# Yotsuei/ClearConverse

Measured on AMD Instinct MI355X. Metric: xRT (audio-sec/wall-sec) end-to-end, 30 s 16 kHz clips, higher is better.
Workload: dtype bf16

## Files before the change

clearconverse_amd/_lib.py:

```python
from __future__ import annotations

import ctypes as C
import os
from pathlib import Path
from typing import Optional

_PKG = Path(__file__).resolve().parent
LIB_PATH = _PKG / "libccx.so"


class CcxError(RuntimeError):
    pass


class WhisperDims(C.Structure):
    _fields_ = [(n, C.c_int) for n in (
        "n_mels", "n_audio_ctx", "n_audio_state", "n_audio_head", "n_audio_layer",
        "n_vocab", "n_text_ctx", "n_text_state", "n_text_head", "n_text_layer")]


class SepformerDims(C.Structure):
    _fields_ = [(n, C.c_int) for n in (
        "n_filters", "kernel", "stride", "d_model", "n_head", "d_ffn", "n_layers", "n_blocks", "segment", "n_spk")]

# ... 31 lines not shown
        ("rows", C.c_int), ("n_seq", C.c_int), ("H", C.c_int), ("kv_T", C.c_int), ("T", C.c_int),
        ("pos", C.POINTER(C.c_int)), ("row_seq", C.POINTER(C.c_int)), ("rows_per_seq", C.c_int),
        ("nsplit", C.c_int), ("combine", C.c_int), ("lds_pad", C.c_int),
        ("x", C.c_void_p), ("pend", C.c_void_p), ("pend_n", C.c_int), ("pend_stride", C.c_int64),
        ("ln_g", C.c_void_p), ("ln_b", C.c_void_p), ("eps", C.c_float),
        ("wq_host", C.c_void_p), ("bq", C.c_void_p),
        ("out", C.c_void_p), ("part_o", C.c_void_p), ("part_ml", C.c_void_p), ("q_x_out", C.c_void_p),
        ("q_elems", C.c_int64), ("kv_elems", C.c_int64), ("out_elems", C.c_int64), ("part_o_elems", C.c_int64),
        ("part_ml_elems", C.c_int64), ("x_elems", C.c_int64), ("pend_elems", C.c_int64), ("q_x_out_elems", C.c_int64),
        ("ind", C.POINTER(C.c_uint16)), ("ind_ld", C.c_int)]


DEC_ATTN_SELF, DEC_ATTN_SPLIT, DEC_ATTN_STREAM, DEC_ATTN_PREFILL, DEC_ATTN_FUSED_Q, DEC_ATTN_TWO_LAUNCH_Q = range(6)
DEC_ATTN_STREAM_MAPPED = 7
DEC_ATTN_SELF_IND = 8


class DecodeSamplingOptions(C.Structure):
    _fields_ = [("top_k", C.c_int), ("top_p", C.c_float), ("min_p", C.c_float)]


class DecSeqState(C.Structure):
    _fields_ = [(n, C.c_int) for n in ("pos", "prompt_len", "n_gen", "done", "last_tok", "pen_tok", "last_ts_tok", "n_tokens")] + [
        ("sum_logprob", C.c_float), ("no_speech_prob", C.c_float)]


class DecSelectDesc(C.Structure):
    _fields_ = [
        ("logits", C.c_void_p), ("ld", C.c_int64), ("n_vocab", C.c_int), ("B", C.c_int),
        ("rules", C.POINTER(DecodeRules)), ("state", C.POINTER(DecSeqState)),
# ... 208 lines not shown
    "ccx_whisper_set_history_options": (_i, [_vp, C.POINTER(DecodeHistoryOptions)]),
    "ccx_whisper_history_graph_count": (_i, [_vp]),
    "ccx_dec_history_step": (_i, [_vp, C.POINTER(DecHistoryDesc), _vp]),
    "ccx_decode_bias_options_default": (None, [C.POINTER(DecodeBiasOptions)]),
    "ccx_whisper_set_bias_options": (_i, [_vp, C.POINTER(DecodeBiasOptions)]),
    "ccx_whisper_bias_graph_count": (_i, [_vp]),
    "ccx_dec_bias_step": (_i, [_vp, C.POINTER(DecBiasDesc), _vp]),
    "ccx_decode_sampling_options_default": (None, [C.POINTER(DecodeSamplingOptions)]),
    "ccx_whisper_set_sampling_options": (_i, [_vp, C.POINTER(DecodeSamplingOptions)]),
    "ccx_whisper_sampling_graph_count": (_i, [_vp]),
    "ccx_whisper_set_mel": (_i, [_vp, _vp, _i, _vp]),
    "ccx_whisper_encode": (_i, [_vp, _i, _vp, _vp]),
    "ccx_whisper_decoder_logits": (_i, [_vp, _i32p, _i, _i, _vp, _vp]),
    "ccx_whisper_decode_greedy": (_i, [_vp, _i32p, _i32p, _i, _i, _i, _i32p, _i32p, _fp, _fp, _vp]),
    "ccx_dec_attention_desc": (_i, [_vp, _i, C.POINTER(DecAttnDesc), _vp]),
    "ccx_dec_select_step": (_i, [_vp, C.POINTER(DecSelectDesc), _vp]),
    "ccx_dec_beam_step": (_i, [_vp, C.POINTER(DecBeamDesc), _vp]),
    "ccx_whisper_decode_beam": (_i, [_vp, _i32p, _i32p, _i, _i, _i32p, _i, _i, _i, _i, _i32p, _i32p, _fp, _i32p, _fp,
                                     C.POINTER(BeamTrace), _vp]),
    "ccx_dec_token_probs": (_i, [_vp, C.POINTER(DecTokenProbsDesc), _vp]),
    "ccx_dec_pick_probs": (_i, [_vp, C.POINTER(DecPickProbsDesc), _vp]),
    "ccx_align_op": (_i, [_vp, _i, C.POINTER(AlignDesc), _vp]),
    "ccx_whisper_align": (_i, [_vp, _i32p, _i32p, _i, _i, _i32p, _i32p, _i, _i, _vp, _vp, _i32p, _vp]),
    "ccx_whisper_align_probs": (_i, [_vp, _i32p, _i32p, _i, _i, _i32p, _i32p, _i, _i, _vp, _vp, _i32p, _i, _fp, _vp]),
    "ccx_whisper_last_cross_path": (_i, [_vp]),
    "ccx_whisper_set_sot_tail": (_i, [_vp, _i]),
    "ccx_whisper_set_prefix_len": (_i, [_vp, _i]),
    "ccx_whisper_detect_language": (_i, [_vp, _i, _i, _i, _i32p, _fp, _vp]),
    "ccx_whisper_prepare_lanes": (_i, [_vp, _vp]),
    "ccx_whisper_trace_lanes": (_i, [_vp, C.c_char_p, _i]),
# ... 118 lines not shown
```

clearconverse_amd/csrc/dec_ops.hip:

```cpp
#include "../../include/ccx.h"
#include "ccx_common.h"
#include "decoder.h"
#include "op_scratch.h"

static_assert(sizeof(ccx_dec_seq_state) == sizeof(DecSeqState), "ccx_dec_seq_state mirrors DecSeqState field for field");

namespace {

__global__ void dec_ops_bf16_to_f32_kernel(const bf16_t* __restrict__ in, float* __restrict__ out, long n) {
  const long i = (long)blockIdx.x * 256 + threadIdx.x;
  if (i < n) out[i] = bf16_to_f32(in[i]);
}

}

extern "C" int ccx_dec_attention_desc(ccx_ctx* ctx, int form, const ccx_dec_attn_desc* d, void* stream_) {
  if (!ctx) return CCX_ERR_ARG;
  hipStream_t stream = (hipStream_t)stream_;
  CCX_REQUIRE(ctx, d != nullptr, "ccx_dec_attention_desc: desc is NULL");
  CCX_REQUIRE(ctx, (form >= CCX_DEC_ATTN_SELF && form <= CCX_DEC_ATTN_TWO_LAUNCH_Q) || form == CCX_DEC_ATTN_STREAM_MAPPED || form == CCX_DEC_ATTN_SELF_IND,
              "ccx_dec_attention_desc: unknown form %d", form);
  const bool is_ind = form == CCX_DEC_ATTN_SELF_IND;
  const bool is_self = form == CCX_DEC_ATTN_SELF || is_ind, is_split = form == CCX_DEC_ATTN_SPLIT, is_mapped = form == CCX_DEC_ATTN_STREAM_MAPPED,
             is_stream = form == CCX_DEC_ATTN_STREAM || is_mapped;
// ... 120 lines not shown
    rc = ccx_launch_dec_cross_fused_q(ctx, ap, rows, nsplit, stream);
  } else {
    DO_HIP(sc.alloc(&d_q, (size_t)rows * 768));
    DecLinearParams lp;
    memset(&lp, 0, sizeof(lp));
    lp.M = rows; lp.N = 768; lp.K = 768; lp.W = d_wq; lp.ldw = 768; lp.bias = (const float*)d->bq; lp.out = d_q; lp.ldo = 768;
    lp.x = (const float*)d->x; lp.pend = (const float*)d->pend; lp.pend_n = d->pend_n; lp.pend_stride = (long)d->pend_stride;
    lp.x_out = (float*)d->q_x_out; lp.ln_g = (const float*)d->ln_g; lp.ln_b = (const float*)d->ln_b; lp.eps = d->eps;
    rc = ccx_launch_dec_linear(ctx, ACT_LN, DEPI_F32, lp, stream);
    ap.q = d_q;
    if (rc == CCX_OK) rc = ccx_launch_dec_attention(ctx, ap, rows, nsplit, false, stream);
  }
  if (rc == CCX_OK && final_out) {
    hipLaunchKernelGGL(dec_ops_bf16_to_f32_kernel, dim3((unsigned)((n_out + 255) / 256)), dim3(256), 0, stream, d_out16, (float*)d->out, n_out);
    DO_HIP(hipGetLastError());
  }
  DO_HIP(hipStreamSynchronize(stream));
  return rc;
}

extern "C" int ccx_dec_select_step(ccx_ctx* ctx, const ccx_dec_select_desc* d, void* stream_) {
  if (!ctx) return CCX_ERR_ARG;
  hipStream_t stream = (hipStream_t)stream_;
  CCX_REQUIRE(ctx, d != nullptr, "ccx_dec_select_step: desc is NULL");
  const int V = d->n_vocab, B = d->B, D = d->D;
  CCX_REQUIRE(ctx, B >= 1 && B <= 65536, "ccx_dec_select_step: B = %d out of range", B);
  CCX_REQUIRE(ctx, V >= 4 && V % 4 == 0 && V <= 13 * 4096, "ccx_dec_select_step: n_vocab = %d must be a multiple of 4 and <= 53248", V);
  CCX_REQUIRE(ctx, d->ld >= V && d->ld % 4 == 0, "ccx_dec_select_step: ld = %ld must be >= n_vocab and a multiple of 4", (long)d->ld);
  CCX_REQUIRE(ctx, d->logits && ccx_aligned16(d->logits), "ccx_dec_select_step: logits null or not 16-byte aligned");
  CCX_REQUIRE(ctx, (int64_t)(B - 1) * d->ld + V <= d->logits_elems, "ccx_dec_select_step: logits are read up to element %ld, logits_elems=%ld",
// ... 226 lines not shown
```

clearconverse_amd/csrc/decoder.h:

```cpp
#pragma once
#include <cstring>
#include <vector>
#include "../../include/ccx.h"
#include "ccx_common.h"

enum { ACT_LN = 0, ACT_BF16 = 1, ACT_COMBINE = 2 };
enum { DEPI_BF16_GELU = 1, DEPI_PARTIAL = 2, DEPI_F32 = 3, DEPI_SELF_QKV = 4, DEPI_RESOLVE = 5 };

struct DecLinearParams {
  int M, N, K;
  const bf16_t* W; long ldw;
  const float* bias;
  const float* x;
  const float* pend; int pend_n; long pend_stride;
  float* x_out;
  const float* ln_g; const float* ln_b; float eps;
  float* ln_mean_out;
  const bf16_t* act; long lda;
  const float* part_o; const float* part_ml; int nsplit;
  float* xres; bf16_t* xb; float2* st_out; const float* shift; float shift_c;
  void* out; long ldo;
  bf16_t* cache_k; bf16_t* cache_v; int cache_T; const int* pos; const int* row_seq;
};
int ccx_launch_dec_linear(ccx_ctx* ctx, int act, int epi, const DecLinearParams& p, hipStream_t stream);
int ccx_dec_linear_ksplit(int K, int epi);
int ccx_launch_dec_resolve_ln(ccx_ctx* ctx, const float* x, const float* pend, int pend_n, long pend_stride, const float* g,
                              const float* b, bf16_t* out, float* x_out, int M, int K, float eps, hipStream_t stream,
                              float* mean_out = nullptr);

struct DecAttnParams {
  const float* q;
  const bf16_t* k;
  const bf16_t* v;
  int H, kv_T;
  const int* pos;
  int T;
  float scale_log2e;
  bf16_t* out_bf16;
  float* part_o;
  float* part_ml;
  int lds_pad;
  int stream_mode;
  const int* row_seq; int rows_per_seq;
// ... 172 lines not shown
```

clearconverse_amd/csrc/decoder.hip:

```cpp
#include <string>
#include "decoder.h"

__global__ void dec_embed_kernel(const float* __restrict__ tok_emb, const float* __restrict__ pos_emb,
                                 const int* __restrict__ cur_tok, const int* __restrict__ pos, float* __restrict__ x,
                                 int D) {
  const int b = blockIdx.x;
  const float4* te = (const float4*)(tok_emb + (long)cur_tok[b] * D);
  const float4* pe = (const float4*)(pos_emb + (long)pos[b] * D);
  float4* xo = (float4*)(x + (long)b * D);
  for (int i = threadIdx.x; i < D / 4; i += blockDim.x) {
    const float4 a = te[i], c = pe[i];
    xo[i] = make_float4(a.x + c.x, a.y + c.y, a.z + c.z, a.w + c.w);
  }
}

#include "dec_ln.h"

__device__ __forceinline__ float centre_shift(float mean, float rstd) { return fabsf(mean) * rstd > 1.f ? mean : 0.f; }

__device__ __forceinline__ uint4 combine_partials(const float* part_o, const float* part_ml, int nsplit, int mh, int c) {
  const float2* ml = (const float2*)(part_ml + ((long)mh * nsplit) * 2);
  const float* ob = part_o + ((long)mh * nsplit) * 64 + 8 * c;
  float2 mlv[8];
  float4 oa[8], oc[8];
// ... 89 lines not shown
  }

  bf16x8 wf[NT][KMAX];
#pragma unroll
  for (int i = 0; i < NT; i++) {
    const long tile = (long)(blockIdx.x * NT + i) * ksteps + ks0;
    const bf16_t* wr = p.W + (tile * 64 + lane) * 8;
#pragma unroll
    for (int k = 0; k < KMAX; k++) {
      const int kk = k < nks ? k : 0;
      wf[i][k] = __builtin_nontemporal_load((const bf16x8*)(wr + 512 * kk));
    }
  }
  bf16x8 af[MT][KMAX];
  if (BF16IN) {
#pragma unroll
    for (int j = 0; j < MT; j++) {
      int m = m0 + 16 * j + l15;
      m = m < p.M ? m : p.M - 1;
      const bf16_t* ar = p.act + (long)m * p.lda + 8 * h4 + 32 * ks0;
#pragma unroll
      for (int k = 0; k < KMAX; k++) {
        const int kk = k < nks ? k : 0;
        af[j][k] = *(const bf16x8*)(ar + 32 * kk);
      }
    }
  }

  if (ACT == ACT_LN) {
    const int nv = K >> 2;
    int live = p.M - m0;
    live = live > MROWS ? MROWS : live;
    const bool writer = (blockIdx.x == 0 && blockIdx.z == 0 && p.x_out != nullptr);
    float4 g[LNS], bb[LNS];
#pragma unroll
    for (int i = 0; i < LNS; i++) {
      const int idx = lane + 64 * i;
      const int ic = idx < nv ? idx : 0;
      g[i] = ((const float4*)p.ln_g)[ic];
// ... 119 lines not shown
        *(float4*)(p.xres + (long)m * p.N + n) = make_float4(v[0], v[1], v[2], v[3]);
        uint2 pk;
        pk.x = pack_bf16x2(c0, c1); pk.y = pack_bf16x2(c2, c3);
        *(uint2*)(p.xb + (long)m * p.N + n) = pk;
        if ((ln >> 4) == 0) p.st_out[(long)m * (p.N >> 4) + (n >> 4)] = make_float2(s1, s2);
      }
      continue;
    }
    if (n >= p.N || m >= p.M) continue;
    f32x4 v = *(const f32x4*)(red + (((0 * NT + i) * MT + j) * 64 + ln) * 4);
#pragma unroll
    for (int w = 1; w < NW; w++) v += *(const f32x4*)(red + (((w * NT + i) * MT + j) * 64 + ln) * 4);
    v[0] += bias_v[it].x; v[1] += bias_v[it].y; v[2] += bias_v[it].z; v[3] += bias_v[it].w;
    const bool full = n + 3 < p.N;
    if (EPI == DEPI_BF16_GELU) {
      bf16_t* o = (bf16_t*)p.out + (long)m * p.ldo + n;
      if (full) {
        uint2 pk;
        pk.x = pack_bf16x2(gelu_erf(v[0]), gelu_erf(v[1]));
        pk.y = pack_bf16x2(gelu_erf(v[2]), gelu_erf(v[3]));
        *(uint2*)o = pk;
      } else {
        for (int c = 0; c < 4 && n + c < p.N; c++) o[c] = f32_to_bf16(gelu_erf(v[c]));
      }
    } else if (EPI == DEPI_PARTIAL || EPI == DEPI_F32) {
      float* o = (float*)p.out + (EPI == DEPI_PARTIAL ? (long)blockIdx.z * p.pend_stride : 0L) + (long)m * p.ldo + n;
      if (full) *(float4*)o = make_float4(v[0], v[1], v[2], v[3]);
      else
        for (int c = 0; c < 4 && n + c < p.N; c++) o[c] = v[c];
    } else if (EPI == DEPI_SELF_QKV) {
      const int D = p.K;
// ... 8 lines not shown
        const int sq = p.row_seq ? p.row_seq[m] : m;
        uint2 pk;
        pk.x = pack_bf16x2(v[0], v[1]);
        pk.y = pack_bf16x2(v[2], v[3]);
        *(uint2*)(cache + (((long)sq * H + hh) * p.cache_T + pos_v[it]) * 64 + d) = pk;
      }
    }
  }
}

template <int NS>
__global__ __launch_bounds__(256) void dec_resolve_ln_kernel(const float* __restrict__ x, const float* __restrict__ pend,
                                                             int pend_n, long pend_stride, const float* __restrict__ g,
                                                             const float* __restrict__ b, bf16_t* __restrict__ out,
                                                             float* __restrict__ x_out, int M, int K, float eps,
                                                             float* __restrict__ mean_out) {
  const int lane = threadIdx.x & 63;
  const int m = blockIdx.x * 4 + (threadIdx.x >> 6);
  if (m >= M) return;
  const int nv = K >> 2;
  float4 v[NS], gg[NS], bb[NS];
#pragma unroll
  for (int i = 0; i < NS; i++) {
    const int idx = lane + 64 * i;
    const int ic = idx < nv ? idx : 0;
    gg[i] = ((const float4*)g)[ic];
    bb[i] = ((const float4*)b)[ic];
  }
  float sm = 0.f;
#pragma unroll
  for (int i = 0; i < NS; i++) {
// ... 10 lines not shown
    if (x_out && idx < nv) ((float4*)(x_out + (long)m * K))[idx] = a;
    sm += ln_sum4(a);
  }
  const float mean = wave_reduce_sum(sm) / (float)K;
  float sq = 0.f;
#pragma unroll
  for (int i = 0; i < NS; i++) {
    const float t = ln_sq4(v[i], mean);
    sq += (lane + 64 * i < nv) ? t : 0.f;
  }
  const float rstd = rsqrtf(wave_reduce_sum(sq) / (float)K + eps);
  if (mean_out && lane == 0) mean_out[m] = centre_shift(mean, rstd);
#pragma unroll
  for (int i = 0; i < NS; i++) {
    const int idx = lane + 64 * i;
    if (idx < nv) ((uint2*)(out + (long)m * K))[idx] = ln_pack4(v[i], mean, rstd, gg[i], bb[i]);
  }
}

__global__ __launch_bounds__(256) void dec_combine_kernel(const float* __restrict__ part_o, const float* __restrict__ part_ml,
                                                          int nsplit, bf16_t* __restrict__ out, int M, int H) {
  const int e = blockIdx.x * 256 + threadIdx.x;
  if (e >= M * H * 8) return;
  const int c = e & 7, h = (e >> 3) % H, m = e / (8 * H);
  *(uint4*)(out + ((long)m * H + h) * 64 + 8 * c) = combine_partials(part_o, part_ml, nsplit, m * H + h, c);
}

__global__ void dec_gather_rows_kernel(const bf16_t* __restrict__ src, const int* __restrict__ idx, bf16_t* __restrict__ dst, int D) {
  if (idx[blockIdx.x] < 0) return;
  const uint4* s4 = (const uint4*)(src + (long)idx[blockIdx.x] * D);
  uint4* d4 = (uint4*)(dst + (long)blockIdx.x * D);
// ... 6 lines not shown
  CCX_CHECK_LAUNCH(ctx);
  return CCX_OK;
}

int ccx_launch_dec_combine(ccx_ctx* ctx, const float* part_o, const float* part_ml, int nsplit, bf16_t* out, int M, int H,
                           hipStream_t stream) {
  CCX_REQUIRE(ctx, nsplit >= 1 && nsplit <= 8, "dec_combine: nsplit out of range");
  ccx_prof_scope ps(ctx, stream, "dec_combine_kernel", 0.0, (double)M * H * nsplit * 66.0 * 4 + (double)M * H * 64 * 2);
  hipLaunchKernelGGL(dec_combine_kernel, dim3(ccx_cdiv(M * H * 8, 256)), dim3(256), 0, stream, part_o, part_ml, nsplit, out, M, H);
  CCX_CHECK_LAUNCH(ctx);
  return CCX_OK;
}

int ccx_launch_dec_resolve_ln(ccx_ctx* ctx, const float* x, const float* pend, int pend_n, long pend_stride, const float* g,
                              const float* b, bf16_t* out, float* x_out, int M, int K, float eps, hipStream_t stream,
                              float* mean_out) {
  CCX_REQUIRE(ctx, K % 4 == 0 && K <= 1280, "dec_resolve_ln: K=%d unsupported (a multiple of 4, at most 1280)", K);
  CCX_REQUIRE(ctx, x_out != x, "dec_resolve_ln: x_out must not alias x");
  ccx_prof_scope ps(ctx, stream, "dec_resolve_ln_kernel", 0.0, (double)M * K * (4.0 * (1 + pend_n) + 2.0 + (x_out ? 4.0 : 0.0)));
  if (K <= 1024)
    hipLaunchKernelGGL(dec_resolve_ln_kernel<4>, dim3(ccx_cdiv(M, 4)), dim3(256), 0, stream, x, pend, pend_n, pend_stride, g, b,
                       out, x_out, M, K, eps, mean_out);
  else
    hipLaunchKernelGGL(dec_resolve_ln_kernel<5>, dim3(ccx_cdiv(M, 4)), dim3(256), 0, stream, x, pend, pend_n, pend_stride, g, b,
                       out, x_out, M, K, eps, mean_out);
  CCX_CHECK_LAUNCH(ctx);
  return CCX_OK;
}

template <int MT, int NT, int KMAX, int ACT, int EPI>
static int launch_dec_linear_inst(ccx_ctx* ctx, const DecLinearParams& p, int ksplit, hipStream_t stream) {
  const int MROWS = 16 * MT, BN = 16 * NT;
  size_t act_bytes = ACT == ACT_BF16 ? 0 : ccx_align((size_t)MROWS * (p.K + 8) * 2, 16);
  size_t red_bytes = (size_t)4 * NT * MT * 64 * 4 * 4;
  size_t lds = act_bytes + red_bytes;
  CCX_REQUIRE(ctx, lds <= 160 * 1024, "dec_linear: LDS %zu too large", lds);
  CCX_REQUIRE(ctx, ccx_cdiv(ccx_cdiv(p.K / 32, ksplit), 4) <= KMAX, "dec_linear: K=%d / split %d exceeds the prefetch depth %d", p.K, ksplit, KMAX);
  if (EPI == DEPI_RESOLVE) CCX_REQUIRE(ctx, p.xres && p.xb && p.st_out && ksplit == 1 && p.N % BN == 0, "dec_linear: bad resolve arguments (N=%d, %d columns per block)", p.N, BN);
  static ccx_lds_optin optin;
  if (lds > 64 * 1024) CCX_HIP(ctx, optin.ensure(ctx->device, (const void*)dec_linear_kernel<MT, NT, KMAX, ACT, EPI>));
// ... 16 lines not shown
  if (need <= 6) {
    if (M <= 16) return launch_dec_linear_inst<1, NT, 6, ACT, EPI>(ctx, p, ksplit, stream);
    if (M <= 32) return launch_dec_linear_inst<2, NT, 6, ACT, EPI>(ctx, p, ksplit, stream);
    return launch_dec_linear_inst<4, NT, 6, ACT, EPI>(ctx, p, ksplit, stream);
  }
  if (need <= 8) {
    if (M <= 16) return launch_dec_linear_inst<1, NT, 8, ACT, EPI>(ctx, p, ksplit, stream);
    if (M <= 32) return launch_dec_linear_inst<2, NT, 8, ACT, EPI>(ctx, p, ksplit, stream);
    return launch_dec_linear_inst<4, NT, 8, ACT, EPI>(ctx, p, ksplit, stream);
  }
  if (M <= 16) return launch_dec_linear_inst<1, NT, 10, ACT, EPI>(ctx, p, ksplit, stream);
  if (M <= 32) return launch_dec_linear_inst<2, NT, 10, ACT, EPI>(ctx, p, ksplit, stream);
  return launch_dec_linear_inst<4, NT, 10, ACT, EPI>(ctx, p, ksplit, stream);
}

int ccx_dec_linear_ksplit(int K, int epi) {
  if (epi == DEPI_RESOLVE) return 1;
  int ks = ccx_cdiv(K, 1024);
  if (epi != DEPI_PARTIAL) return K <= 1280 ? 1 : ks;
  if (ks > 4) ks = ccx_cdiv(K, 1280);
  return ks < 1 ? 1 : ks;
}

int ccx_launch_dec_linear(ccx_ctx* ctx, int act, int epi, const DecLinearParams& p, hipStream_t stream) {
  CCX_REQUIRE(ctx, p.M > 0 && p.N > 0 && p.K > 0 && p.K % 32 == 0, "dec_linear: bad shape M=%d N=%d K=%d", p.M, p.N, p.K);
  CCX_REQUIRE(ctx, act == ACT_BF16 || p.K <= 1280, "dec_linear: LN/combine activation needs K <= 1280");
  CCX_REQUIRE(ctx, p.pend_n >= 0 && p.pend_n <= 4, "dec_linear: at most 4 pending slabs");
  const int ksplit = ccx_dec_linear_ksplit(p.K, epi);
  CCX_REQUIRE(ctx, epi == DEPI_PARTIAL || ksplit == 1, "dec_linear: K=%d needs a split-K (partial) epilogue", p.K);
  CCX_REQUIRE(ctx, ksplit <= 4, "dec_linear: K=%d would leave %d partial slabs (at most 4)", p.K, ksplit);
  CCX_REQUIRE(ctx, epi != DEPI_PARTIAL || p.pend_stride >= (long)p.M * p.ldo, "dec_linear: pend_stride too small");
  if (epi == DEPI_RESOLVE) {
    CCX_REQUIRE(ctx, act == ACT_BF16, "dec_linear: the resolve epilogue takes bf16 activations");
    if (p.M >= 128) return launch_dec_linear_mt<2, ACT_BF16, DEPI_RESOLVE>(ctx, p, 1, stream);
    return launch_dec_linear_mt<1, ACT_BF16, DEPI_RESOLVE>(ctx, p, 1, stream);
  }
  if (p.M >= 128 && act == ACT_BF16) {
    if (epi == DEPI_PARTIAL) return launch_dec_linear_mt<2, ACT_BF16, DEPI_PARTIAL>(ctx, p, ksplit, stream);
    if (epi == DEPI_F32) return launch_dec_linear_mt<2, ACT_BF16, DEPI_F32>(ctx, p, 1, stream);
    if (epi == DEPI_SELF_QKV) return launch_dec_linear_mt<2, ACT_BF16, DEPI_SELF_QKV>(ctx, p, 1, stream);
    if (epi == DEPI_BF16_GELU) return launch_dec_linear_mt<2, ACT_BF16, DEPI_BF16_GELU>(ctx, p, 1, stream);
  }
// ... 845 lines not shown
```

clearconverse_amd/csrc/whisper.hip:

```cpp
#include <algorithm>
#include <atomic>
#include <map>
#include <chrono>
#include <math.h>
#include <tuple>
#include "../../include/ccx.h"
#include "align.h"
#include "attention.h"
#include "ccx_common.h"
#include "cross_x.h"
#include "decoder.h"
#include "elementwise.h"
#include "gemm_bf16.h"
#include "logmel.h"
#include "model_store.h"

namespace {

struct EncLayer {
  float *ln1_g, *ln1_b, *ln2_g, *ln2_b;
  bf16_t *Wqkv, *Wo, *W1, *W2;
  float *bqkv, *bo, *b1, *b2;
};
struct DecLayer {
// ... 4 lines not shown
  bf16_t* Wcq_g = nullptr;
  float *scq = nullptr, *ccq = nullptr;
  float bo_mean = 0.f;
  float *bqkv, *bo, *bcq, *bckv, *bco, *b1, *b2;
  bf16_t *crossK, *crossV, *selfK, *selfV;
};

struct StepPlan {
  int b0, B;
  int sample_len, max_prompt;
  int select;
  int sampling;
  int cross_stream;
  int cross_lds_pad;
  int xs_active;
  int lnfree, xs_fuse_q, fuse_cross_q, xs_full_lines;
  int map_on, sid_on;
  int beam_size, beam_maxc;
  int lane_idx;
  int stamp_level;
  int prefill_rows;
  int opt_mask;
  int no_ts;
  int sup_blank;
  int max_init_ts;
  int hist_ngram;
  int hist_pen_bits;
  int bias_on;
  int trunc_on;
  auto tie() const {
    return std::tie(b0, B, sample_len, max_prompt, select, sampling, cross_stream, cross_lds_pad, xs_active, lnfree, xs_fuse_q, fuse_cross_q,
                    xs_full_lines, map_on, sid_on, beam_size, beam_maxc, lane_idx, stamp_level, prefill_rows, opt_mask, no_ts, sup_blank,
                    max_init_ts, hist_ngram, hist_pen_bits, bias_on, trunc_on);
  }
  bool operator<(const StepPlan& o) const { return tie() < o.tie(); }
};
static_assert(sizeof(StepPlan) == 28 * sizeof(int) && std::tuple_size<decltype(StepPlan{}.tie())>::value == 28,
              "StepPlan: ints only, and every one of them in tie()");

}

struct ccx_whisper {
  ccx_ctx* ctx = nullptr;
  ccx_whisper_dims d{};
  int max_batch = 0;
  bool finalized = false;
  ccx_whisper* scratch_donor = nullptr;
  int scratch_takers = 0;
  bool destroy_pending = false;
  std::atomic<ccx_whisper*> scratch_owner{nullptr};
  hipEvent_t scratch_free = nullptr;
  ccx_dev_store store{"whisper"};
// ... 671 lines not shown
    const DecLayer& L = w->dec[l];
    memset(&p, 0, sizeof(p));
    p.A = w->xa; p.lda = D; p.W = L.Wckv; p.ldw = D; p.M = n * S; p.N = 2 * D; p.K = D; p.bias = L.bckv;
    p.hk = L.crossK; p.hv = L.crossV; p.d_model = D; p.n_head = H; p.S = S; p.Spad = w->Spad; p.v_transposed = 0;
    p.first_block = 1;
    CCX_TRY(ccx_launch_gemm(w->ctx, EPI_HEADS, p, stream));
  }
  w->kv_ready = n;
  return CCX_OK;
}
static void read_chain_switches(StepPlan& p) {
  { const char* e = getenv("CCX_FUSE_CROSS_Q"); p.fuse_cross_q = e ? (atoi(e) != 0) : 1; }
  { const char* e = getenv("CCX_DEC_LNFREE"); p.lnfree = !(e && strcmp(e, "0") == 0); }
  { const char* e = getenv("CCX_XS_FUSE_Q"); p.xs_fuse_q = !e || atoi(e) != 0; }
  p.xs_full_lines = ccx_xs_full_lines_switch();
}
static int select_cross_path(ccx_whisper* w, StepPlan& p, hipStream_t stream, int n_kv = -1) {
  const int B = p.B;
  const char* e = getenv("CCX_CROSS_X_MIN_ROWS");
  const int min_rows = e ? atoi(e) : ccx_whisper::kKvSeqs + 1;
  if (n_kv < 0) n_kv = B;
  p.xs_active = w->xs_on && (B >= min_rows || n_kv > w->kv_cap);
  if (w->xs_on && !p.xs_active && w->kv_ready < n_kv) CCX_TRY(project_cross_kv(w, n_kv, stream));
  return CCX_OK;
}
static StepPlan single_lane_plan(const ccx_whisper* w, int B, int max_prompt) {
  StepPlan p{};
  p.B = B; p.sample_len = 1; p.max_prompt = max_prompt; p.cross_stream = 1;
  p.stamp_level = w->stamps_on ? w->stamp_level : 0;
  read_chain_switches(p);
// ... 208 lines not shown
  float* dq = pre ? w->pf_q : w->dq + ro * D;
  bf16_t* dxn = pre ? w->pf_xn : w->dxn + ro * D;
  bf16_t* dattn = pre ? w->pf_attn : w->dattn + ro * D;
  bf16_t* dffn = pre ? w->pf_ffn : w->dffn + ro * F;
  float* part_o = w->part_o + ro * H * ccx_whisper::kCrossSplitMax * 64;
  float* part_ml = w->part_ml + ro * H * ccx_whisper::kCrossSplitMax * 2;
  int* pos = pre ? w->pf_pos : w->pos + b0;
  const int* row_seq = pre ? w->pf_seq : nullptr;
  const int* win = !map_on ? nullptr : (pre ? w->pf_win : w->row_win + b0);
  const long cross_off = map_on ? 0 : ro * H * w->Spad * 64, self_off = ro * H * Tc * 64;
  auto stamp = [&](int tag, int level) {
    if (level <= p.stamp_level)
      hipLaunchKernelGGL(dec_stamp_kernel, dim3(1), dim3(1), 0, stream, w->stamps + (size_t)lane_idx * ccx_whisper::kStampCap,
                         w->stamp_count + lane_idx, ccx_whisper::kStampCap, tag);
  };
  int pend_n = 0;
  auto ln_linear = [&](int epi, const bf16_t* W, const float* bias, int N, const float* g, const float* bta, void* out, long ldo,
                       DecLinearParams* extra) -> int {
    DecLinearParams lp;
    if (extra) lp = *extra; else memset(&lp, 0, sizeof(lp));
    lp.M = B; lp.N = N; lp.K = D; lp.W = W; lp.ldw = D; lp.bias = bias; lp.out = out; lp.ldo = ldo;
    int rc;
    if (B > 16) {
      rc = ccx_launch_dec_resolve_ln(ctx, cur, pend, pend_n, pstride, g, bta, dxn, pend_n > 0 ? other : nullptr, B, D, 1e-5f, stream,
                                     lp.ln_mean_out);
      if (rc) return rc;
      lp.ln_mean_out = nullptr;
      lp.act = dxn; lp.lda = D;
      rc = ccx_launch_dec_linear(ctx, ACT_BF16, epi, lp, stream);
    } else {
      lp.x = cur; lp.pend = pend; lp.pend_n = pend_n; lp.pend_stride = pstride; lp.x_out = pend_n > 0 ? other : nullptr;
      lp.ln_g = g; lp.ln_b = bta; lp.eps = 1e-5f;
      rc = ccx_launch_dec_linear(ctx, ACT_LN, epi, lp, stream);
    }
    if (rc) return rc;
    if (pend_n > 0) { float* t = cur; cur = other; other = t; pend_n = 0; }
    return CCX_OK;
  };
  auto partial_linear = [&](int act, const bf16_t* W, const float* bias, int K, const bf16_t* a) -> int {
    DecLinearParams lp;
    memset(&lp, 0, sizeof(lp));
    lp.M = B; lp.N = D; lp.K = K; lp.W = W; lp.ldw = K; lp.bias = bias; lp.act = a; lp.lda = K;
    lp.part_o = part_o; lp.part_ml = part_ml; lp.nsplit = ns;
    lp.out = pend; lp.ldo = D; lp.pend_stride = pstride;
    int rc = ccx_launch_dec_linear(ctx, act, DEPI_PARTIAL, lp, stream);
    if (rc) return rc;
    pend_n = ccx_dec_linear_ksplit(K, DEPI_PARTIAL);
    return CCX_OK;
  };
  const bool lnfree = xs_active && p.lnfree;
  const bool xs_fused = xs_active && !lnfree && p.xs_fuse_q;
  const bool fuse_q = !xs_active && p.fuse_cross_q && !pre && B <= 16 && D == 768 && !map_on;
  const bool q_launch = !fuse_q && !lnfree && !xs_fused;
  bf16_t* xb = !lnfree ? nullptr : (pre ? w->pf_xb : w->dxb + ro * D);
  float2* st2 = !lnfree ? nullptr : (pre ? w->pf_st2 : w->dst2 + ro * (D / 16));
  float* shift = !lnfree ? nullptr : (pre ? w->pf_shift : w->dshift + ro);
  for (int l = 0; l < d.n_text_layer; l++) {
// ... 69 lines not shown
        ap.rows_per_seq = prefill_rows > 1 ? prefill_rows : 0;
        ap.lds_pad = 0; ap.stream_mode = 1;
        CCX_TRY(ccx_launch_dec_attention(ctx, ap, nseq, 1, true, stream));
        CCX_TRY(partial_linear(ACT_BF16, L.Wco, L.bco, D, dattn));
      } else if (B > 16) {
        CCX_TRY(ccx_launch_dec_attention(ctx, ap, B, ns, ns == 1, stream));
        stamp(2, 1);
        if (ns > 1) CCX_TRY(ccx_launch_dec_combine(ctx, part_o, part_ml, ns, dattn, B, H, stream));
        CCX_TRY(partial_linear(ACT_BF16, L.Wco, L.bco, D, dattn));
        stamp(19, 2);
      } else {
        CCX_TRY(ccx_launch_dec_attention(ctx, ap, B, ns, false, stream));
        CCX_TRY(partial_linear(ACT_COMBINE, L.Wco, L.bco, D, nullptr));
      }
    }
    CCX_TRY(ln_linear(DEPI_BF16_GELU, L.W1, L.b1, F, L.ln2_g, L.ln2_b, dffn, F, nullptr));
    stamp(20, 2);
    CCX_TRY(partial_linear(ACT_BF16, L.W2, L.b2, F, dffn));
    stamp(21, 2);
  }
  CCX_TRY(ccx_launch_dec_resolve_ln(ctx, cur, pend, pend_n, pstride, w->lnd_g, w->lnd_b, dxn, nullptr, B, D, 1e-5f, stream));
  if (pre) return CCX_OK;
  CCX_TRY(dec_head(w, p, io));
  stamp(3, 1);
  return CCX_OK;
}

int upload_decode_state(ccx_whisper* w, const int32_t* prompt_ids, const int32_t* prompt_lens, int max_prompt, int B,
                        float temperature, uint64_t seed, hipStream_t stream, bool prefilled = false) {
  std::vector<DecSeqState> st(B);
  std::vector<int> tok(B), ps(B, 0);
  for (int b = 0; b < B; b++) {
    memset(&st[b], 0, sizeof(DecSeqState));
// ... 787 lines not shown
```

include/ccx.h:

```cpp
#ifndef CCX_H
#define CCX_H
#include <stdint.h>
#ifdef __cplusplus
extern "C" {
#endif

#define CCX_DTYPE_F32 0
#define CCX_DTYPE_BF16 1
#define CCX_DTYPE_F16 2

typedef struct ccx_ctx ccx_ctx;
typedef struct ccx_whisper ccx_whisper;

const char* ccx_version(void);
int ccx_ctx_create(int device, ccx_ctx** out);
void ccx_ctx_destroy(ccx_ctx* ctx);
const char* ccx_last_error(const ccx_ctx* ctx);

int ccx_prof_enable(ccx_ctx* ctx, int on);
int ccx_prof_count(ccx_ctx* ctx);
int ccx_prof_get(ccx_ctx* ctx, int i, char* name_out, int name_cap, double* flops, double* bytes, float* ms);


int ccx_gemm_bf16(ccx_ctx* ctx, int epi, const void* A_dev, int64_t lda, const void* W_dev, int64_t ldw,
// ... 185 lines not shown
  int sample_len;
  int* gen;
  int* cur_tok; int* pos;
  int* n_done;
  const void* tok_emb; const void* pos_emb; void* x; int D;
  int sample; float temperature; uint64_t seed; int row0;
  int64_t logits_elems, tok_emb_elems, pos_emb_elems, x_elems;
  const int* stream_ids;
  const ccx_decode_options* opts;
  const ccx_decode_sampling_options* sampling;
  float* cut_out; int* kept_out; float* kept_mass_out;
} ccx_dec_select_desc;

int ccx_dec_select_step(ccx_ctx* ctx, const ccx_dec_select_desc* desc, void* stream);

typedef struct ccx_dec_beam_desc {
  const void* logits; int64_t ld; int n_vocab;
  int G, beam_size, max_candidates;
  const ccx_decode_rules* rules;
  ccx_dec_seq_state* state;
  int sample_len;
  int* hist; int* cur_tok; int* pos; int* n_done;
  const void* tok_emb; const void* pos_emb; void* x; int D;
  uint16_t* ind; int ind_ld;
  int* fin_tok; float* fin_score; int* fin_n; int* fin_count;
  int* cand_id; float* cand_lp; int* tok_out; int* parent_out;
  int64_t logits_elems, tok_emb_elems, pos_emb_elems, x_elems;
  const ccx_decode_options* opts;
} ccx_dec_beam_desc;
int ccx_dec_beam_step(ccx_ctx* ctx, const ccx_dec_beam_desc* desc, void* stream);
// ... 245 lines not shown
```

Measured before the change: 1772.

## Write decoder LN and GELU activations in MFMA fragment-packed layout

```diff
diff --git a/clearconverse_amd/_lib.py b/clearconverse_amd/_lib.py
--- a/clearconverse_amd/_lib.py
+++ b/clearconverse_amd/_lib.py
@@ -69,6 +69,14 @@
 DEC_ATTN_SELF, DEC_ATTN_SPLIT, DEC_ATTN_STREAM, DEC_ATTN_PREFILL, DEC_ATTN_FUSED_Q, DEC_ATTN_TWO_LAUNCH_Q = range(6)
 DEC_ATTN_STREAM_MAPPED = 7
 DEC_ATTN_SELF_IND = 8
+
+
+class DecLnLinearDesc(C.Structure):
+    _fields_ = [
+        ("M", C.c_int), ("K", C.c_int), ("F", C.c_int), ("N", C.c_int), ("epi", C.c_int), ("packed", C.c_int),
+        ("x", C.c_void_p), ("ln_g", C.c_void_p), ("ln_b", C.c_void_p), ("eps", C.c_float),
+        ("w1_host", C.c_void_p), ("b1", C.c_void_p), ("w_host", C.c_void_p), ("bias", C.c_void_p),
+        ("out", C.c_void_p), ("x_elems", C.c_int64), ("out_elems", C.c_int64)]
 
 
 class DecodeSamplingOptions(C.Structure):
@@ -307,6 +315,7 @@
     "ccx_whisper_decoder_logits": (_i, [_vp, _i32p, _i, _i, _vp, _vp]),
     "ccx_whisper_decode_greedy": (_i, [_vp, _i32p, _i32p, _i, _i, _i, _i32p, _i32p, _fp, _fp, _vp]),
     "ccx_dec_attention_desc": (_i, [_vp, _i, C.POINTER(DecAttnDesc), _vp]),
+    "ccx_dec_ln_linear": (_i, [_vp, C.POINTER(DecLnLinearDesc), _vp]),
     "ccx_dec_select_step": (_i, [_vp, C.POINTER(DecSelectDesc), _vp]),
     "ccx_dec_beam_step": (_i, [_vp, C.POINTER(DecBeamDesc), _vp]),
     "ccx_whisper_decode_beam": (_i, [_vp, _i32p, _i32p, _i, _i, _i32p, _i, _i, _i, _i, _i32p, _i32p, _fp, _i32p, _fp,
diff --git a/clearconverse_amd/csrc/dec_ops.hip b/clearconverse_amd/csrc/dec_ops.hip
--- a/clearconverse_amd/csrc/dec_ops.hip
+++ b/clearconverse_amd/csrc/dec_ops.hip
@@ -158,6 +158,103 @@
   if (rc == CCX_OK && final_out) {
     hipLaunchKernelGGL(dec_ops_bf16_to_f32_kernel, dim3((unsigned)((n_out + 255) / 256)), dim3(256), 0, stream, d_out16, (float*)d->out, n_out);
     DO_HIP(hipGetLastError());
+  }
+  DO_HIP(hipStreamSynchronize(stream));
+  return rc;
+}
+
+namespace {
+
+__global__ void dec_ops_rows_to_f32_kernel(const bf16_t* __restrict__ in, float* __restrict__ out, int M, int K, int packed) {
+  const long i = (long)blockIdx.x * 256 + threadIdx.x;
+  if (i >= (long)M * K) return;
+  const int m = (int)(i / K), k = (int)(i - (long)m * K);
+  out[i] = bf16_to_f32(in[packed ? dec_frag_off(m, k, K >> 5) : i]);
+}
+
+}
+
+extern "C" int ccx_dec_ln_linear(ccx_ctx* ctx, const ccx_dec_ln_linear_desc* d, void* stream_) {
+  if (!ctx) return CCX_ERR_ARG;
+  hipStream_t stream = (hipStream_t)stream_;
+  CCX_REQUIRE(ctx, d != nullptr, "ccx_dec_ln_linear: desc is NULL");
+  const int M = d->M, K = d->K, F = d->F, N = d->N, epi = d->epi, packed = d->packed;
+  CCX_REQUIRE(ctx, M >= 1 && M <= 4096, "ccx_dec_ln_linear: M = %d out of range [1, 4096]", M);
+  CCX_REQUIRE(ctx, K >= 32 && K % 32 == 0 && K <= 1280, "ccx_dec_ln_linear: K = %d must be a multiple of 32 in [32, 1280]", K);
+  CCX_REQUIRE(ctx, F == 0 || (F >= 32 && F % 32 == 0 && F <= 5120), "ccx_dec_ln_linear: F = %d must be 0 or a multiple of 32 up to 5120", F);
+  CCX_REQUIRE(ctx, N >= 4 && N % 4 == 0 && N <= 8192, "ccx_dec_ln_linear: N = %d must be a multiple of 4 in [4, 8192]", N);
+  CCX_REQUIRE(ctx, epi >= CCX_DEC_EPI_PARTIAL && epi <= CCX_DEC_EPI_GELU, "ccx_dec_ln_linear: unknown epi %d", epi);
+  CCX_REQUIRE(ctx, packed == 0 || packed == 1, "ccx_dec_ln_linear: packed = %d must be 0 or 1", packed);
+  CCX_REQUIRE(ctx, epi != CCX_DEC_EPI_SELF_QKV || (F == 0 && K % 64 == 0 && N == 3 * K), "ccx_dec_ln_linear: SELF_QKV needs F == 0, K a multiple of 64 and N == 3 K");
+  CCX_REQUIRE(ctx, epi != CCX_DEC_EPI_GELU || N % 32 == 0, "ccx_dec_ln_linear: the GELU epilogue needs N = %d to be a multiple of 32", N);
+  const int Kin = F > 0 ? F : K;
+  const int depi = epi == CCX_DEC_EPI_PARTIAL ? DEPI_PARTIAL : epi == CCX_DEC_EPI_F32 ? DEPI_F32 : epi == CCX_DEC_EPI_SELF_QKV ? DEPI_SELF_QKV : DEPI_BF16_GELU;
+  const int ksplit = ccx_dec_linear_ksplit(Kin, depi);
+  CCX_REQUIRE(ctx, epi == CCX_DEC_EPI_PARTIAL || ksplit == 1, "ccx_dec_ln_linear: %d input columns need the PARTIAL epilogue", Kin);
+  CCX_REQUIRE(ctx, ksplit <= 4, "ccx_dec_ln_linear: %d input columns leave %d slabs (at most 4)", Kin, ksplit);
+  CCX_REQUIRE(ctx, d->x && d->ln_g && d->ln_b && d->w_host && d->out, "ccx_dec_ln_linear: x, ln_g, ln_b, w_host or out is NULL");
+  CCX_REQUIRE(ctx, F == 0 || d->w1_host, "ccx_dec_ln_linear: w1_host is NULL with F = %d", F);
+  CCX_REQUIRE(ctx, ccx_aligned16(d->x) && ccx_aligned16(d->ln_g) && ccx_aligned16(d->ln_b) && ccx_aligned16(d->out) && ccx_aligned16(d->b1) && ccx_aligned16(d->bias),
+              "ccx_dec_ln_linear: x, ln_g, ln_b, b1, bias or out not 16-byte aligned");
+  CCX_REQUIRE(ctx, (int64_t)M * K <= d->x_elems, "ccx_dec_ln_linear: x is read up to element %ld, x_elems=%ld", (long)M * K, (long)d->x_elems);
+  const int64_t n_out = epi == CCX_DEC_EPI_PARTIAL ? (int64_t)ksplit * M * N : epi == CCX_DEC_EPI_SELF_QKV ? (int64_t)3 * M * K : (int64_t)M * N;
+  CCX_REQUIRE(ctx, n_out <= d->out_elems, "ccx_dec_ln_linear: out is written up to element %ld, out_elems=%ld", (long)n_out, (long)d->out_elems);
+
+  ccx_op_scratch sc;
+  const size_t Mp = (size_t)(M + 15) / 16 * 16;
+  bf16_t *d_xn = nullptr, *d_ffn = nullptr, *d_w1 = nullptr, *d_w = nullptr, *d_g16 = nullptr, *d_ck = nullptr, *d_cv = nullptr;
+  float* d_pend = nullptr; int* d_pos = nullptr;
+  DO_HIP(sc.alloc(&d_xn, Mp * K));
+  DO_HIP(hipMemsetAsync(d_xn, 0xFF, Mp * K * 2, stream));
+  DO_HIP(sc.alloc(&d_pend, (size_t)M * K));
+  DO_HIP(hipMemsetAsync(d_pend, 0, (size_t)M * K * 4, stream));
+  DO_HIP(hipMemsetAsync(d->out, 0xFF, (size_t)n_out * 4, stream));
+  {
+    const std::vector<bf16_t> pw = pack_mfma_rows(d->w_host, N, Kin, 32);
+    DO_HIP(sc.upload(&d_w, pw.data(), pw.size()));
+  }
+  int rc = ccx_launch_dec_resolve_ln(ctx, (const float*)d->x, d_pend, 0, (long)M * K, (const float*)d->ln_g, (const float*)d->ln_b, d_xn, nullptr, M, K,
+                                     d->eps, stream, nullptr, packed);
+  const bf16_t* act = d_xn;
+  if (rc == CCX_OK && F > 0) {
+    const std::vector<bf16_t> pw1 = pack_mfma_rows(d->w1_host, F, K, 32);
+    DO_HIP(sc.upload(&d_w1, pw1.data(), pw1.size()));
+    DO_HIP(sc.alloc(&d_ffn, Mp * F));
+    DO_HIP(hipMemsetAsync(d_ffn, 0xFF, Mp * F * 2, stream));
+    DecLinearParams lp;
+    memset(&lp, 0, sizeof(lp));
+    lp.M = M; lp.N = F; lp.K = K; lp.W = d_w1; lp.ldw = K; lp.bias = (const float*)d->b1; lp.act = d_xn; lp.lda = K; lp.act_packed = packed;
+    lp.out = d_ffn; lp.ldo = F; lp.out_packed = packed;
+    rc = ccx_launch_dec_linear(ctx, ACT_BF16, DEPI_BF16_GELU, lp, stream);
+    act = d_ffn;
+  }
+  if (rc == CCX_OK) {
+    DecLinearParams lp;
+    memset(&lp, 0, sizeof(lp));
+    lp.M = M; lp.N = N; lp.K = Kin; lp.W = d_w; lp.ldw = Kin; lp.bias = (const float*)d->bias; lp.act = act; lp.lda = Kin; lp.act_packed = packed;
+    lp.out = d->out; lp.ldo = N; lp.pend_stride = (long)M * N;
+    if (epi == CCX_DEC_EPI_SELF_QKV) {
+      const std::vector<int> pos((size_t)M, 0);
+      DO_HIP(sc.upload(&d_pos, pos.data(), pos.size()));
+      DO_HIP(sc.alloc(&d_ck, (size_t)M * K)); DO_HIP(sc.alloc(&d_cv, (size_t)M * K));
+      DO_HIP(hipMemsetAsync(d_ck, 0xFF, (size_t)M * K * 2, stream)); DO_HIP(hipMemsetAsync(d_cv, 0xFF, (size_t)M * K * 2, stream));
+      lp.ldo = K; lp.cache_k = d_ck; lp.cache_v = d_cv; lp.cache_T = 1; lp.pos = d_pos;
+    } else if (epi == CCX_DEC_EPI_GELU) {
+      DO_HIP(sc.alloc(&d_g16, Mp * N));
+      DO_HIP(hipMemsetAsync(d_g16, 0xFF, Mp * N * 2, stream));
+      lp.out = d_g16; lp.out_packed = packed;
+    }
+    rc = ccx_launch_dec_linear(ctx, ACT_BF16, depi, lp, stream);
+    if (rc == CCX_OK && epi == CCX_DEC_EPI_SELF_QKV) {
+      const long n = (long)M * K;
+      hipLaunchKernelGGL(dec_ops_rows_to_f32_kernel, dim3((unsigned)((n + 255) / 256)), dim3(256), 0, stream, d_ck, (float*)d->out + n, M, K, 0);
+      hipLaunchKernelGGL(dec_ops_rows_to_f32_kernel, dim3((unsigned)((n + 255) / 256)), dim3(256), 0, stream, d_cv, (float*)d->out + 2 * n, M, K, 0);
+      DO_HIP(hipGetLastError());
+    } else if (rc == CCX_OK && epi == CCX_DEC_EPI_GELU) {
+      const long n = (long)M * N;
+      hipLaunchKernelGGL(dec_ops_rows_to_f32_kernel, dim3((unsigned)((n + 255) / 256)), dim3(256), 0, stream, d_g16, (float*)d->out, M, N, packed);
+      DO_HIP(hipGetLastError());
+    }
   }
   DO_HIP(hipStreamSynchronize(stream));
   return rc;
diff --git a/clearconverse_amd/csrc/decoder.h b/clearconverse_amd/csrc/decoder.h
--- a/clearconverse_amd/csrc/decoder.h
+++ b/clearconverse_amd/csrc/decoder.h
@@ -21,12 +21,18 @@
   float* xres; bf16_t* xb; float2* st_out; const float* shift; float shift_c;
   void* out; long ldo;
   bf16_t* cache_k; bf16_t* cache_v; int cache_T; const int* pos; const int* row_seq;
+  int act_packed, out_packed;
 };
 int ccx_launch_dec_linear(ccx_ctx* ctx, int act, int epi, const DecLinearParams& p, hipStream_t stream);
 int ccx_dec_linear_ksplit(int K, int epi);
 int ccx_launch_dec_resolve_ln(ccx_ctx* ctx, const float* x, const float* pend, int pend_n, long pend_stride, const float* g,
                               const float* b, bf16_t* out, float* x_out, int M, int K, float eps, hipStream_t stream,
-                              float* mean_out = nullptr);
+                              float* mean_out = nullptr, int out_packed = 0);
+
+__host__ __device__ __forceinline__ long dec_frag_off(int m, int k, int ksteps) {
+  return (((long)(m >> 4) * ksteps + (k >> 5)) * 64 + (((k >> 3) & 3) * 16 + (m & 15))) * 8 + (k & 7);
+}
+int ccx_dec_packed_act_switch();
 
 struct DecAttnParams {
   const float* q;
diff --git a/clearconverse_amd/csrc/decoder.hip b/clearconverse_amd/csrc/decoder.hip
--- a/clearconverse_amd/csrc/decoder.hip
+++ b/clearconverse_amd/csrc/decoder.hip
@@ -127,15 +127,18 @@
   }
   bf16x8 af[MT][KMAX];
   if (BF16IN) {
+    const int kstride = p.act_packed ? 512 : 32;
 #pragma unroll
     for (int j = 0; j < MT; j++) {
       int m = m0 + 16 * j + l15;
       m = m < p.M ? m : p.M - 1;
-      const bf16_t* ar = p.act + (long)m * p.lda + 8 * h4 + 32 * ks0;
+      int mt = blockIdx.y * MT + j;
+      mt = mt <= ((p.M - 1) >> 4) ? mt : ((p.M - 1) >> 4);
+      const bf16_t* ar = p.act_packed ? p.act + (((long)mt * ksteps + (nks > 0 ? ks0 : 0)) * 64 + lane) * 8 : p.act + (long)m * p.lda + 8 * h4 + 32 * ks0;
 #pragma unroll
       for (int k = 0; k < KMAX; k++) {
         const int kk = k < nks ? k : 0;
-        af[j][k] = *(const bf16x8*)(ar + 32 * kk);
+        af[j][k] = *(const bf16x8*)(ar + kstride * kk);
       }
     }
   }
@@ -285,7 +288,7 @@
     v[0] += bias_v[it].x; v[1] += bias_v[it].y; v[2] += bias_v[it].z; v[3] += bias_v[it].w;
     const bool full = n + 3 < p.N;
     if (EPI == DEPI_BF16_GELU) {
-      bf16_t* o = (bf16_t*)p.out + (long)m * p.ldo + n;
+      bf16_t* o = (bf16_t*)p.out + (BF16IN && p.out_packed ? dec_frag_off(m, n, p.N >> 5) : (long)m * p.ldo + n);
       if (full) {
         uint2 pk;
         pk.x = pack_bf16x2(gelu_erf(v[0]), gelu_erf(v[1]));
@@ -324,7 +327,7 @@
                                                              int pend_n, long pend_stride, const float* __restrict__ g,
                                                              const float* __restrict__ b, bf16_t* __restrict__ out,
                                                              float* __restrict__ x_out, int M, int K, float eps,
-                                                             float* __restrict__ mean_out) {
+                                                             float* __restrict__ mean_out, int out_packed) {
   const int lane = threadIdx.x & 63;
   const int m = blockIdx.x * 4 + (threadIdx.x >> 6);
   if (m >= M) return;
@@ -365,7 +368,7 @@
 #pragma unroll
   for (int i = 0; i < NS; i++) {
     const int idx = lane + 64 * i;
-    if (idx < nv) ((uint2*)(out + (long)m * K))[idx] = ln_pack4(v[i], mean, rstd, gg[i], bb[i]);
+    if (idx < nv) *(uint2*)(out + (out_packed ? dec_frag_off(m, 4 * idx, K >> 5) : (long)m * K + 4 * idx)) = ln_pack4(v[i], mean, rstd, gg[i], bb[i]);
   }
 }
 
@@ -402,16 +405,17 @@
 
 int ccx_launch_dec_resolve_ln(ccx_ctx* ctx, const float* x, const float* pend, int pend_n, long pend_stride, const float* g,
                               const float* b, bf16_t* out, float* x_out, int M, int K, float eps, hipStream_t stream,
-                              float* mean_out) {
+                              float* mean_out, int out_packed) {
   CCX_REQUIRE(ctx, K % 4 == 0 && K <= 1280, "dec_resolve_ln: K=%d unsupported (a multiple of 4, at most 1280)", K);
+  CCX_REQUIRE(ctx, !out_packed || K % 32 == 0, "dec_resolve_ln: the fragment image needs K=%d to be a multiple of 32", K);
   CCX_REQUIRE(ctx, x_out != x, "dec_resolve_ln: x_out must not alias x");
   ccx_prof_scope ps(ctx, stream, "dec_resolve_ln_kernel", 0.0, (double)M * K * (4.0 * (1 + pend_n) + 2.0 + (x_out ? 4.0 : 0.0)));
   if (K <= 1024)
     hipLaunchKernelGGL(dec_resolve_ln_kernel<4>, dim3(ccx_cdiv(M, 4)), dim3(256), 0, stream, x, pend, pend_n, pend_stride, g, b,
-                       out, x_out, M, K, eps, mean_out);
+                       out, x_out, M, K, eps, mean_out, out_packed);
   else
     hipLaunchKernelGGL(dec_resolve_ln_kernel<5>, dim3(ccx_cdiv(M, 4)), dim3(256), 0, stream, x, pend, pend_n, pend_stride, g, b,
-                       out, x_out, M, K, eps, mean_out);
+                       out, x_out, M, K, eps, mean_out, out_packed);
   CCX_CHECK_LAUNCH(ctx);
   return CCX_OK;
 }
@@ -458,6 +462,11 @@
   return launch_dec_linear_inst<4, NT, 10, ACT, EPI>(ctx, p, ksplit, stream);
 }
 
+int ccx_dec_packed_act_switch() {
+  const char* e = getenv("CCX_DEC_PACKED_ACT");
+  return !(e && strcmp(e, "0") == 0);
+}
+
 int ccx_dec_linear_ksplit(int K, int epi) {
   if (epi == DEPI_RESOLVE) return 1;
   int ks = ccx_cdiv(K, 1024);
@@ -470,6 +479,8 @@
   CCX_REQUIRE(ctx, p.M > 0 && p.N > 0 && p.K > 0 && p.K % 32 == 0, "dec_linear: bad shape M=%d N=%d K=%d", p.M, p.N, p.K);
   CCX_REQUIRE(ctx, act == ACT_BF16 || p.K <= 1280, "dec_linear: LN/combine activation needs K <= 1280");
   CCX_REQUIRE(ctx, p.pend_n >= 0 && p.pend_n <= 4, "dec_linear: at most 4 pending slabs");
+  CCX_REQUIRE(ctx, !p.act_packed || act == ACT_BF16, "dec_linear: act_packed is taken with bf16 activations only");
+  CCX_REQUIRE(ctx, !p.out_packed || (act == ACT_BF16 && epi == DEPI_BF16_GELU && p.N % 32 == 0), "dec_linear: out_packed needs the GELU epilogue and N=%d a multiple of 32", p.N);
   const int ksplit = ccx_dec_linear_ksplit(p.K, epi);
   CCX_REQUIRE(ctx, epi == DEPI_PARTIAL || ksplit == 1, "dec_linear: K=%d needs a split-K (partial) epilogue", p.K);
   CCX_REQUIRE(ctx, ksplit <= 4, "dec_linear: K=%d would leave %d partial slabs (at most 4)", p.K, ksplit);
diff --git a/clearconverse_amd/csrc/whisper.hip b/clearconverse_amd/csrc/whisper.hip
--- a/clearconverse_amd/csrc/whisper.hip
+++ b/clearconverse_amd/csrc/whisper.hip
@@ -42,7 +42,7 @@
   int cross_stream;
   int cross_lds_pad;
   int xs_active;
-  int lnfree, xs_fuse_q, fuse_cross_q, xs_full_lines;
+  int lnfree, xs_fuse_q, fuse_cross_q, xs_full_lines, packed_act;
   int map_on, sid_on;
   int beam_size, beam_maxc;
   int lane_idx;
@@ -58,12 +58,12 @@
   int trunc_on;
   auto tie() const {
     return std::tie(b0, B, sample_len, max_prompt, select, sampling, cross_stream, cross_lds_pad, xs_active, lnfree, xs_fuse_q, fuse_cross_q,
-                    xs_full_lines, map_on, sid_on, beam_size, beam_maxc, lane_idx, stamp_level, prefill_rows, opt_mask, no_ts, sup_blank,
+                    xs_full_lines, packed_act, map_on, sid_on, beam_size, beam_maxc, lane_idx, stamp_level, prefill_rows, opt_mask, no_ts, sup_blank,
                     max_init_ts, hist_ngram, hist_pen_bits, bias_on, trunc_on);
   }
   bool operator<(const StepPlan& o) const { return tie() < o.tie(); }
 };
-static_assert(sizeof(StepPlan) == 28 * sizeof(int) && std::tuple_size<decltype(StepPlan{}.tie())>::value == 28,
+static_assert(sizeof(StepPlan) == 29 * sizeof(int) && std::tuple_size<decltype(StepPlan{}.tie())>::value == 29,
               "StepPlan: ints only, and every one of them in tie()");
 
 }
@@ -765,6 +765,7 @@
   { const char* e = getenv("CCX_DEC_LNFREE"); p.lnfree = !(e && strcmp(e, "0") == 0); }
   { const char* e = getenv("CCX_XS_FUSE_Q"); p.xs_fuse_q = !e || atoi(e) != 0; }
   p.xs_full_lines = ccx_xs_full_lines_switch();
+  p.packed_act = ccx_dec_packed_act_switch();
 }
 static int select_cross_path(ccx_whisper* w, StepPlan& p, hipStream_t stream, int n_kv = -1) {
   const int B = p.B;
@@ -1003,6 +1004,7 @@
       hipLaunchKernelGGL(dec_stamp_kernel, dim3(1), dim3(1), 0, stream, w->stamps + (size_t)lane_idx * ccx_whisper::kStampCap,
                          w->stamp_count + lane_idx, ccx_whisper::kStampCap, tag);
   };
+  const int packed = (p.packed_act && B > 16 && B % 16 == 0) ? 1 : 0;
   int pend_n = 0;
   auto ln_linear = [&](int epi, const bf16_t* W, const float* bias, int N, const float* g, const float* bta, void* out, long ldo,
                        DecLinearParams* extra) -> int {
@@ -1012,10 +1014,10 @@
     int rc;
     if (B > 16) {
       rc = ccx_launch_dec_resolve_ln(ctx, cur, pend, pend_n, pstride, g, bta, dxn, pend_n > 0 ? other : nullptr, B, D, 1e-5f, stream,
-                                     lp.ln_mean_out);
+                                     lp.ln_mean_out, packed);
       if (rc) return rc;
       lp.ln_mean_out = nullptr;
-      lp.act = dxn; lp.lda = D;
+      lp.act = dxn; lp.lda = D; lp.act_packed = packed;
       rc = ccx_launch_dec_linear(ctx, ACT_BF16, epi, lp, stream);
     } else {
       lp.x = cur; lp.pend = pend; lp.pend_n = pend_n; lp.pend_stride = pstride; lp.x_out = pend_n > 0 ? other : nullptr;
@@ -1026,10 +1028,10 @@
     if (pend_n > 0) { float* t = cur; cur = other; other = t; pend_n = 0; }
     return CCX_OK;
   };
-  auto partial_linear = [&](int act, const bf16_t* W, const float* bias, int K, const bf16_t* a) -> int {
+  auto partial_linear = [&](int act, const bf16_t* W, const float* bias, int K, const bf16_t* a, int a_packed = 0) -> int {
     DecLinearParams lp;
     memset(&lp, 0, sizeof(lp));
-    lp.M = B; lp.N = D; lp.K = K; lp.W = W; lp.ldw = K; lp.bias = bias; lp.act = a; lp.lda = K;
+    lp.M = B; lp.N = D; lp.K = K; lp.W = W; lp.ldw = K; lp.bias = bias; lp.act = a; lp.lda = K; lp.act_packed = a_packed;
     lp.part_o = part_o; lp.part_ml = part_ml; lp.nsplit = ns;
     lp.out = pend; lp.ldo = D; lp.pend_stride = pstride;
     int rc = ccx_launch_dec_linear(ctx, act, DEPI_PARTIAL, lp, stream);
@@ -1129,9 +1131,14 @@
         CCX_TRY(partial_linear(ACT_COMBINE, L.Wco, L.bco, D, nullptr));
       }
     }
-    CCX_TRY(ln_linear(DEPI_BF16_GELU, L.W1, L.b1, F, L.ln2_g, L.ln2_b, dffn, F, nullptr));
+    {
+      DecLinearParams ex;
+      memset(&ex, 0, sizeof(ex));
+      ex.out_packed = packed;
+      CCX_TRY(ln_linear(DEPI_BF16_GELU, L.W1, L.b1, F, L.ln2_g, L.ln2_b, dffn, F, &ex));
+    }
     stamp(20, 2);
-    CCX_TRY(partial_linear(ACT_BF16, L.W2, L.b2, F, dffn));
+    CCX_TRY(partial_linear(ACT_BF16, L.W2, L.b2, F, dffn, packed));
     stamp(21, 2);
   }
   CCX_TRY(ccx_launch_dec_resolve_ln(ctx, cur, pend, pend_n, pstride, w->lnd_g, w->lnd_b, dxn, nullptr, B, D, 1e-5f, stream));
diff --git a/include/ccx.h b/include/ccx.h
--- a/include/ccx.h
+++ b/include/ccx.h
@@ -223,6 +223,20 @@
 
 int ccx_dec_select_step(ccx_ctx* ctx, const ccx_dec_select_desc* desc, void* stream);
 
+#define CCX_DEC_EPI_PARTIAL 0
+#define CCX_DEC_EPI_F32 1
+#define CCX_DEC_EPI_SELF_QKV 2
+#define CCX_DEC_EPI_GELU 3
+typedef struct ccx_dec_ln_linear_desc {
+  int M, K, F, N, epi, packed;
+  const void* x; const void* ln_g; const void* ln_b; float eps;
+  const float* w1_host; const void* b1;
+  const float* w_host; const void* bias;
+  void* out;
+  int64_t x_elems, out_elems;
+} ccx_dec_ln_linear_desc;
+int ccx_dec_ln_linear(ccx_ctx* ctx, const ccx_dec_ln_linear_desc* desc, void* stream);
+
 typedef struct ccx_dec_beam_desc {
   const void* logits; int64_t ld; int n_vocab;
   int G, beam_size, max_candidates;
```

Result: faster. 1809 (median of 6 runs) (+2.1%).
